# integritychain/fips204

Measured on AMD Instinct MI355X. Metric: ML-DSA-65 verifies/sec per GPU (batched); % HBM roofline, higher is better.
Workload: dtype int32; 1 GPU; ml_dsa_65 batch=65536 whole verify on FIPS 204 wire formats; batch_per_gpu=65536, parallelism=batch-split x1

## Files before the change

### fips204_amd/ml_dsa.py

```python
import ctypes as C

import numpy as np
import torch

from . import _keycheck_lib, _keys_lib, _lib, _mu_lib, _mus_lib, _ph_lib, _rec_lib, _seed_lib, _vfy_lib
from .hotpath import HotPath, N, _optr, _ptr, _stream

MODE_PURE, MODE_INTERNAL, MODE_PREHASH = 0, 1, 2

VFY_MIN_OPS = {44: 24576, 65: 16384, 87: 65536}

PH_SHA256, PH_SHA512, PH_SHAKE128 = "SHA256", "SHA512", "SHAKE128"
PH_SHA384, PH_SHA224, PH_SHA512_224, PH_SHA512_256 = "SHA384", "SHA224", "SHA512_224", "SHA512_256"
PH_SHA3_224, PH_SHA3_256, PH_SHA3_384, PH_SHA3_512, PH_SHAKE256 = "SHA3_224", "SHA3_256", "SHA3_384", "SHA3_512", "SHAKE256"
_PH_OID = bytes([0x06, 0x09, 0x60, 0x86, 0x48, 0x01, 0x65, 0x03, 0x04, 0x02])
_PH_TABLE = {
    PH_SHA256: (0x01, "sha256", None, _ph_lib.PH_SHA256),
    PH_SHA384: (0x02, "sha384", None, _ph_lib.PH_SHA384),
    PH_SHA512: (0x03, "sha512", None, _ph_lib.PH_SHA512),
    PH_SHA224: (0x04, "sha224", None, _ph_lib.PH_SHA224),
    PH_SHA512_224: (0x05, "sha512_224", None, _ph_lib.PH_SHA512_224),
    PH_SHA512_256: (0x06, "sha512_256", None, _ph_lib.PH_SHA512_256),
    PH_SHA3_224: (0x07, "sha3_224", None, _ph_lib.PH_SHA3_224),
    PH_SHA3_256: (0x08, "sha3_256", None, _ph_lib.PH_SHA3_256),
    PH_SHA3_384: (0x09, "sha3_384", None, _ph_lib.PH_SHA3_384),
    PH_SHA3_512: (0x0A, "sha3_512", None, _ph_lib.PH_SHA3_512),
    PH_SHAKE128: (0x0B, "shake_128", 32, _ph_lib.PH_SHAKE128),
    PH_SHAKE256: (0x0C, "shake_256", 64, _ph_lib.PH_SHAKE256),
}
_PH_ABI = {name: row[3] for name, row in _PH_TABLE.items()}
_PH_NAMES = "Ph: " + ", ".join(_PH_TABLE)


def _ph_code(ph):
    if ph not in _PH_ABI:
        raise ValueError(_PH_NAMES)
    return _PH_ABI[ph]


def _check_prehash(prehash):
    if prehash not in ("host", "device"):
        raise ValueError('prehash: "host" or "device"')
    return prehash == "device"


class OsRng:

    def fill_bytes(self, n):
        import os
        return os.urandom(n)


def hash_message(message, ph):
    import hashlib
    message = bytes(message)
    if not isinstance(ph, str) or ph not in _PH_TABLE:
        raise ValueError(_PH_NAMES)
    oid_last, name, xof_len, _ = _PH_TABLE[ph]
    h = hashlib.new(name, message)
    return _PH_OID + bytes([oid_last]) + (h.digest(xof_len) if xof_len else h.digest())


def external_mu(tr, message, ctx=b"", mode=MODE_PURE):
    import hashlib
    tr, message, ctx = bytes(tr), bytes(message), bytes(ctx)
    if len(tr) != 64:
        raise ValueError("tr: 64 bytes expected")
    if mode == MODE_INTERNAL:
        m_prime = message
    elif mode in (MODE_PURE, MODE_PREHASH):
        if len(ctx) > 255:
            raise ValueError("ctx too long (at most 255 bytes)")
        m_prime = bytes([1 if mode == MODE_PREHASH else 0, len(ctx)]) + ctx + message
    else:
        raise ValueError("mode: MODE_PURE, MODE_INTERNAL or MODE_PREHASH")
    return hashlib.shake_256(tr + m_prime).digest(64)


FORM_SEED, FORM_EXPANDED, FORM_BOTH = "seed", "expanded", "both"


def private_key_forms(seed=None, expanded=None):
    if seed is None and expanded is None:
        raise ValueError("a private key needs a seed, an expanded key or both")
    for name, key in (("seed", seed), ("expanded key", expanded)):
        if key is not None and not isinstance(key, (bytes, bytearray, memoryview)):
            raise TypeError(f"{name}: bytes, bytearray or memoryview expected, not {type(key).__name__}")
    if seed is not None and memoryview(seed).nbytes != _seed_lib.SEED_LEN:
        raise ValueError(f"seed: {_seed_lib.SEED_LEN} bytes expected")
    if expanded is not None and memoryview(expanded).nbytes == 0:
        raise ValueError("expanded key: empty")
    if expanded is None:
        return FORM_SEED, "expand_seeds"
    if seed is None:
        return FORM_EXPANDED, "sk_expand"
    return FORM_BOTH, "check_then_expand"


_SK_SHAPE = {44: (4, 4, 2), 65: (6, 5, 4), 87: (8, 7, 2)}


def private_key_faults(pset, sk_bytes):
    if pset not in _SK_SHAPE:
        raise ValueError(f"unknown parameter set {pset!r}")
    k, l, eta = _SK_SHAPE[pset]
    bits = 3 if eta == 2 else 4
    sk_len = 128 + 32 * bits * (l + k) + 416 * k
    if isinstance(sk_bytes, (bytes, bytearray, memoryview)):
        sk_bytes = [sk_bytes]
    if isinstance(sk_bytes, np.ndarray):
        a = np.ascontiguousarray(sk_bytes, dtype=np.uint8).reshape(-1)
    else:
        a = np.frombuffer(b"".join(bytes(b) for b in sk_bytes), dtype=np.uint8)
    if a.size % sk_len:
        raise ValueError(f"sk: {a.size} bytes are not a multiple of SK_LEN = {sk_len}")
    a = a.reshape(-1, sk_len)
    region = np.unpackbits(a[:, 128:128 + 32 * bits * (l + k)], axis=1, bitorder="little")
    fields = region.reshape(a.shape[0], (l + k) * 256, bits).astype(np.uint8) @ (1 << np.arange(bits)).astype(np.uint8)
    over = fields > 2 * eta
    return (over[:, :l * 256].any(axis=1) * _keycheck_lib.KEY_S1_RANGE + over[:, l * 256:].any(axis=1) * _keycheck_lib.KEY_S2_RANGE).astype(np.uint8)


def _np_ptr(a):
    return C.c_void_p(0) if a is None else C.c_void_p(a.ctypes.data)


def _cat(items):
    lens = np.fromiter((len(b) for b in items), dtype=np.uint64, count=len(items))
    off = np.zeros(len(items) + 1, dtype=np.uint64)
    np.cumsum(lens, out=off[1:])
    return b"".join(bytes(b) for b in items) or b"\0", off


def _cat_with_offsets(items, device):
    flat, off = _cat(items)
    buf = torch.frombuffer(bytearray(flat), dtype=torch.uint8).to(device)
    return buf, torch.from_numpy(off.view(np.int64)).to(device)


class PublicKeys:

    def __init__(self, pset, rho, tr, t1_d2_hat_mont):
        self.pset, self.rho, self.tr, self.t1_d2_hat_mont = pset, rho, tr, t1_d2_hat_mont

    def __len__(self):
        return self.rho.shape[0]


class PrivateKeys:

    def __init__(self, pset, rho, cap_k, tr, s_1_hat_mont, s_2_hat_mont, t_0_hat_mont):
        self.pset, self.rho, self.cap_k, self.tr = pset, rho, cap_k, tr
        self.s_1_hat_mont, self.s_2_hat_mont, self.t_0_hat_mont = s_1_hat_mont, s_2_hat_mont, t_0_hat_mont

    def __len__(self):
        return self.rho.shape[0]

    def zeroize(self):
        for t in (self.cap_k, self.s_1_hat_mont, self.s_2_hat_mont, self.t_0_hat_mont):
            if t is not None:
                t.zero_()

    def __del__(self):
# ... 1078 lines not shown
```

### fips204_amd/vfy/keccak180.h

```cpp
#pragma once
#include "../csrc/keccak.h"
#include "../csrc/sampler_dev.h"

namespace mldsa_vfy {

using mldsa::KeccakState;

#define VFY_RHOPI(DST, SRC, ROT)                                                                                                  \
    mldsa::rotl64<ROT>(mldsa::xor3(s.lo[SRC], clo[((SRC) + 4) % 5], rlo[((SRC) + 1) % 5]),                                        \
                       mldsa::xor3(s.hi[SRC], chi_[((SRC) + 4) % 5], rhi[((SRC) + 1) % 5]), blo[DST], bhi[DST])

__device__ __forceinline__ void keccak_round180(KeccakState& s, uint32_t rc_lo, uint32_t rc_hi) {
    uint32_t clo[5], chi_[5], rlo[5], rhi[5], blo[25], bhi[25];
#pragma unroll
    for (int x = 0; x < 5; x++) {
        clo[x] = mldsa::xor3(mldsa::xor3(s.lo[x], s.lo[x + 5], s.lo[x + 10]), s.lo[x + 15], s.lo[x + 20]);
        chi_[x] = mldsa::xor3(mldsa::xor3(s.hi[x], s.hi[x + 5], s.hi[x + 10]), s.hi[x + 15], s.hi[x + 20]);
    }
#pragma unroll
    for (int x = 0; x < 5; x++) mldsa::rotl64<1>(clo[x], chi_[x], rlo[x], rhi[x]);
    VFY_RHOPI(0, 0, 0);
    VFY_RHOPI(10, 1, 1);
    VFY_RHOPI(20, 2, 62);
    VFY_RHOPI(5, 3, 28);
    VFY_RHOPI(15, 4, 27);
    VFY_RHOPI(16, 5, 36);
    VFY_RHOPI(1, 6, 44);
    VFY_RHOPI(11, 7, 6);
    VFY_RHOPI(21, 8, 55);
    VFY_RHOPI(6, 9, 20);
    VFY_RHOPI(7, 10, 3);
    VFY_RHOPI(17, 11, 10);
    VFY_RHOPI(2, 12, 43);
    VFY_RHOPI(12, 13, 25);
    VFY_RHOPI(22, 14, 39);
    VFY_RHOPI(23, 15, 41);
    VFY_RHOPI(8, 16, 45);
    VFY_RHOPI(18, 17, 15);
    VFY_RHOPI(3, 18, 21);
    VFY_RHOPI(13, 19, 8);
    VFY_RHOPI(14, 20, 18);
    VFY_RHOPI(24, 21, 2);
    VFY_RHOPI(9, 22, 61);
    VFY_RHOPI(19, 23, 56);
    VFY_RHOPI(4, 24, 14);
#pragma unroll
    for (int y = 0; y < 25; y += 5) {
#pragma unroll
        for (int x = 0; x < 5; x++) {
            s.lo[y + x] = mldsa::chi(blo[y + x], blo[y + (x + 1) % 5], blo[y + (x + 2) % 5]);
            s.hi[y + x] = mldsa::chi(bhi[y + x], bhi[y + (x + 1) % 5], bhi[y + (x + 2) % 5]);
        }
    }
    s.lo[0] ^= rc_lo;
    s.hi[0] ^= rc_hi;
}
#undef VFY_RHOPI

__device__ __forceinline__ void keccak_f1600_180(KeccakState& s) {
#pragma unroll 1
    for (int r = 0; r < 24; r++) {
        const uint32_t rc_lo = mldsa::KECCAK_RC_LO[r];
        const uint32_t rc_hi = ((mldsa::KECCAK_RC_HI_BITS >> r) & 1u) << 31;
        keccak_round180(s, rc_lo, rc_hi);
    }
}

__device__ __forceinline__ void rej_ntt_poly_lane_direct180(KeccakState& st, int32_t* __restrict__ out, size_t wave_base, int lane, bool valid) {
    constexpr uint32_t ROW = mldsa::PACKED_POLY_DWORDS * 4;
    const size_t wb = ((size_t)(uint32_t)__builtin_amdgcn_readfirstlane((int)(wave_base >> 32)) << 32) |
                      (uint32_t)__builtin_amdgcn_readfirstlane((int)(uint32_t)wave_base);
    uint8_t* base = reinterpret_cast<uint8_t*>(out) + wb * ROW;
    const uint32_t end = (uint32_t)(lane + 1) * ROW;
    uint32_t off = valid ? (uint32_t)lane * ROW : end;
    while (__any(off < end)) {
        keccak_f1600_180(st);
        mldsa::static_for<0, 14>([&](auto gc) {
            constexpr int G = decltype(gc)::value;
            const uint32_t m0 = mldsa::state_word<3 * G>(st) & 0xFF7FFFFFu, m1 = mldsa::state_word<3 * G + 1>(st) & 0xFFFF7FFFu,
                           m2 = mldsa::state_word<3 * G + 2>(st) & 0x7FFFFF7Fu;
            const uint64_t lo = (((uint64_t)m1 << 32) | m0) + 0x1FFF001FFF001FFFull;
            const uint32_t hi = m2 + 0x001FFF00u + (uint32_t)(lo < 0x1FFF001FFF001FFFull ? 1u : 0u);
            const uint32_t over = ((uint32_t)lo & 0x00800000u) | ((uint32_t)(lo >> 32) & 0x00008000u) | (hi & 0x80000080u);
            if (over == 0u && off + 12u <= end) {
                *reinterpret_cast<mldsa::Packed3Unaligned*>(base + off) = mldsa::Packed3Unaligned{m0, m1, m2};
                off += 12u;
            } else if (off < end) {
                const uint32_t c[4] = {m0 & 0x7FFFFFu, __builtin_amdgcn_alignbit(m1, m0, 24) & 0x7FFFFFu,
                                       __builtin_amdgcn_alignbit(m2, m1, 16) & 0x7FFFFFu, m2 >> 8};
#pragma unroll
                for (int k = 0; k < 4; k++) {
                    if (c[k] < (uint32_t)mldsa::Q && off < end) {
                        uint8_t* dst = base + off;
                        dst[0] = (uint8_t)c[k];
                        dst[1] = (uint8_t)(c[k] >> 8);
                        dst[2] = (uint8_t)(c[k] >> 16);
                        off += 3u;
                    }
                }
            }
        });
    }
}

}
```

### fips204_amd/vfy/vfy.hip

```cpp
#include <hip/hip_runtime.h>
#include <stdint.h>
#include <string.h>

#include <mutex>
#include <string>
#include <vector>

#include "../../include/mldsa_vfy.h"
#include "../layer/layer_dev.h"
#include "../layer/layer_host.h"
#include "../csrc/challenge_dev.h"
#include "../csrc/ntt_wave.h"
#include "../csrc/sampler_dev.h"
#include "../csrc/tables.h"
#include "../csrc/verify_dev.h"
#include "keccak180.h"
#include "vfy_parts.h"

namespace mldsa_vfy {

using mldsa::FWD_TW;
using mldsa::INV_TW;
using mldsa::N;
using mldsa::SHAKE256_RATE;
// ... 404 lines not shown
        diff |= (st.lo[W] ^ load_le32(c0 + 8 * W)) | (st.hi[W] ^ load_le32(c0 + 8 * W + 4));
    });
    ok[op] = (uint8_t)(diff == 0 && znorm[op] < zbound && hvalid[op] && !ctx_bad[op]);
}

}

namespace {

using namespace mldsa_layer;
using namespace mldsa_vfy;

struct DevState {
    int dev = -1;
    int n_cu = 256;
    hipStream_t ea = nullptr, vm = nullptr;
    std::vector<hipEvent_t> ev;
    Twiddle *fwd = nullptr, *inv = nullptr;
    bool prof_on = false;
    std::vector<hipEvent_t> prof_ev;
    std::vector<const char*> prof_name;
    size_t prof_used = 0;
};

std::mutex g_mutex;
std::vector<DevState*> g_states;
size_t g_part_ops = 0;

size_t part_ops() { return g_part_ops ? g_part_ops : (size_t)MLDSA_VFY_PART_OPS; }

int dev_state(const char* fn, int dev, DevState** out) {
    for (DevState* d : g_states)
        if (d->dev == dev) {
            *out = d;
            return MLDSA_OK;
        }
    DevState* d = new DevState;
    d->dev = dev;
    int cu = 0;
    if (hipDeviceGetAttribute(&cu, hipDeviceAttributeMultiprocessorCount, dev) == hipSuccess && cu > 0) d->n_cu = cu;
    const std::vector<mldsa::HostTwiddle> f = mldsa::gen_fwd_lane_twiddles(), i = mldsa::gen_inv_lane_twiddles();
    hipError_t e = hipStreamCreateWithFlags(&d->ea, hipStreamNonBlocking);
    if (e == hipSuccess) e = hipStreamCreateWithFlags(&d->vm, hipStreamNonBlocking);
    if (e == hipSuccess) e = hipMalloc(&d->fwd, f.size() * sizeof(Twiddle));
    if (e == hipSuccess) e = hipMalloc(&d->inv, i.size() * sizeof(Twiddle));
    if (e == hipSuccess) e = hipMemcpy(d->fwd, f.data(), f.size() * sizeof(Twiddle), hipMemcpyHostToDevice);
    if (e == hipSuccess) e = hipMemcpy(d->inv, i.data(), i.size() * sizeof(Twiddle), hipMemcpyHostToDevice);
    if (e != hipSuccess || f.size() != (size_t)FWD_TW * 64 || i.size() != (size_t)INV_TW * 64) {
        if (d->ea) (void)hipStreamDestroy(d->ea);
        if (d->vm) (void)hipStreamDestroy(d->vm);
        if (d->fwd) (void)hipFree(d->fwd);
        if (d->inv) (void)hipFree(d->inv);
        delete d;
        (void)hipGetLastError();
        return e != hipSuccess ? hip_failed(fn, "creating the library's streams and tables", e)
                               : fail(MLDSA_ERR_DEVICE, std::string(fn) + ": the core's twiddle tables have another shape");
    }
    g_states.push_back(d);
    *out = d;
    return MLDSA_OK;
}

struct Events {
    DevState* d;
    size_t used = 0;
    hipError_t err = hipSuccess;
    explicit Events(DevState* d_) : d(d_) {}
    hipEvent_t next() {
        if (used == d->ev.size()) {
            hipEvent_t e = nullptr;
            const hipError_t rc = hipEventCreateWithFlags(&e, hipEventDisableTiming);
            if (rc != hipSuccess) {
                err = rc;
                return nullptr;
            }
            d->ev.push_back(e);
        }
        return d->ev[used++];
    }
};

constexpr size_t PROF_MAX_PAIRS = 4096;
struct ProfScope {
    DevState* d;
    hipStream_t s;
    long idx = -1;
    ProfScope(DevState* d_, hipStream_t s_, const char* name) : d(d_), s(s_) {
        if (!d->prof_on || d->prof_used >= PROF_MAX_PAIRS) return;
        if (d->prof_used * 2 + 2 > d->prof_ev.size()) {
            hipEvent_t a = nullptr, b = nullptr;
            if (hipEventCreate(&a) != hipSuccess) return;
            if (hipEventCreate(&b) != hipSuccess) {
                (void)hipEventDestroy(a);
                return;
            }
            d->prof_ev.push_back(a);
            d->prof_ev.push_back(b);
            d->prof_name.push_back(name);
        } else {
            d->prof_name[d->prof_used] = name;
        }
        idx = (long)d->prof_used++;
        (void)hipEventRecord(d->prof_ev[2 * idx], s);
    }
    ~ProfScope() {
        if (idx >= 0) (void)hipEventRecord(d->prof_ev[2 * idx + 1], s);
    }
};

#define VFY_HIP(call, what)                                     \
    do {                                                        \
        const hipError_t e_ = (call);                           \
        if (e_ != hipSuccess) return hip_failed(fn, what, e_);  \
    } while (0)

#define VFY_BY_SET(set, M)              \
    do {                                \
        if ((set) == MLDSA_44) M(4, 4, 17, false, 32, 5); \
        else if ((set) == MLDSA_65) M(6, 5, 19, true, 48, 4); \
        else M(8, 7, 19, true, 64, 4);  \
    } while (0)

unsigned stream_blocks(size_t n_streams) { return (unsigned)((n_streams + 64 * SWAVES - 1) / (64 * SWAVES)); }

void launch_expand_a(int set, const uint8_t* rho, const uint32_t* key_idx, int32_t* a_hat, size_t n, uint32_t n_keys, hipStream_t s) {
    mldsa_params p;
    (void)mldsa_get_params(set, &p);
    const dim3 grid(stream_blocks(n * (size_t)(p.k * p.l))), block(64 * SWAVES);
#define VFY_EA(KK, LL, GB, G2, CT, MW) hipLaunchKernelGGL((k_expand_a<KK, LL>), grid, block, 0, s, rho, (size_t)32, key_idx, a_hat, n, n_keys)
    VFY_BY_SET(set, VFY_EA);
#undef VFY_EA
}

struct Call {
    int set, mode;
    mldsa_params p;
    const uint8_t *rho, *tr;
    const int32_t* t1;
    size_t n_keys;
    const uint32_t* key_idx;
    const uint8_t* msgs;
    const uint64_t* msg_off;
    const uint8_t* ctxs;
    const uint64_t* ctx_off;
    const uint8_t* sigs;
    uint8_t* ok;
    size_t n_ops;
};

int enqueue(const char* fn, DevState* d, const Call& c, uint8_t* scratch, hipStream_t s) {
    const mldsa_params& p = c.p;
    const PartPlan plan(c.n_ops, part_ops());
    const Carve cv = carve(p.k, p.l, (size_t)p.w1_len, plan);
    const size_t mw = 64 + (size_t)p.w1_len, n_parts = plan.n_parts();
    uint32_t* c8 = reinterpret_cast<uint32_t*>(scratch + cv.c);
    int32_t* znorm = reinterpret_cast<int32_t*>(scratch + cv.znorm);
    int32_t* hvalid = reinterpret_cast<int32_t*>(scratch + cv.hvalid);
    int32_t* ctx_bad = reinterpret_cast<int32_t*>(scratch + cv.ctx_bad);
    int32_t* key_bad = reinterpret_cast<int32_t*>(scratch + cv.key_bad);
    uint32_t* kidx = reinterpret_cast<uint32_t*>(scratch + cv.kidx);
    uint8_t* mu_w1 = scratch + cv.mu_w1;
    const size_t sig_len = (size_t)p.sig_len;

    Events evs(d);
    hipEvent_t fork = evs.next(), join = evs.next();
    std::vector<hipEvent_t> ready(n_parts), used(n_parts), front(n_parts);
    for (size_t i = 0; i < n_parts; i++) {
        ready[i] = evs.next();
        used[i] = evs.next();
        front[i] = evs.next();
    }
    if (evs.err != hipSuccess) return hip_failed(fn, "creating an event", evs.err);

    VFY_HIP(hipEventRecord(fork, s), "recording the fork");
    VFY_HIP(hipStreamWaitEvent(d->ea, fork, 0), "ordering the ExpandA stream behind the caller's");
    VFY_HIP(hipStreamWaitEvent(d->vm, fork, 0), "ordering the arithmetic stream behind the caller's");
    for (size_t i = 0; i < n_parts; i++) {
        const Part part = plan.at(i);
        const size_t o = part.first, n = part.count;
        const size_t key_base = c.key_idx ? 0 : o;
        int32_t* a_hat = reinterpret_cast<int32_t*>(scratch + cv.ring[part.half]);
        const uint8_t* sg = c.sigs + o * sig_len;
        if (i >= 2) VFY_HIP(hipStreamWaitEvent(d->ea, used[i - 2], 0), "waiting for the ring half");
        {
            ProfScope ps(d, d->ea, "expand_a");
            launch_expand_a(c.set, c.rho + key_base * 32, c.key_idx ? c.key_idx + o : nullptr, a_hat, n, c.key_idx ? (uint32_t)c.n_keys : 0u, d->ea);
        }
        LAYER_LAUNCHED("k_expand_a launch");
        VFY_HIP(hipEventRecord(ready[i], d->ea), "recording ExpandA's end");
        const uint32_t* kp = nullptr;
        const int32_t* kb = nullptr;
        if (c.key_idx) {
            hipLaunchKernelGGL(k_sanitize_keys, dim3((unsigned)((n + 255) / 256)), dim3(256), 0, s, c.key_idx + o, (uint32_t)c.n_keys, n, kidx + o, key_bad + o);
            kp = kidx + o;
            kb = key_bad + o;
        }
        {
            ProfScope ps(d, s, "mu");
            hipLaunchKernelGGL(k_mu, dim3((unsigned)((n + 63) / 64)), dim3(64), 0, s, c.tr + key_base * 64, (size_t)64, kp, c.mode, c.msgs, c.msg_off, c.ctxs,
                               c.ctx_off, mu_w1 + o * mw, mw, ctx_bad + o, kb, n, o, c.n_ops);
        }
        {
            ProfScope ps(d, s, "sample_in_ball");
            const dim3 grid((unsigned)((n + 63) / 64)), block(64);
#define VFY_SIB(KK, LL, GB, G2, CT, MW) hipLaunchKernelGGL((k_sample_in_ball<CT>), grid, block, 0, s, sg, sig_len, p.tau, c8 + o * 64, n)
            VFY_BY_SET(c.set, VFY_SIB);
#undef VFY_SIB
        }
        LAYER_LAUNCHED("front launch");
        VFY_HIP(hipEventRecord(front[i], s), "recording the front's end");
        VFY_HIP(hipStreamWaitEvent(d->vm, ready[i], 0), "waiting for ExpandA");
        VFY_HIP(hipStreamWaitEvent(d->vm, front[i], 0), "waiting for the front");
        {
            ProfScope ps(d, d->vm, "verify_main");
            const size_t need = (n + VW - 1) / VW, cap = (size_t)d->n_cu * 16;
            const dim3 grid((unsigned)(need < cap ? need : cap)), block(64 * VW);
#define VFY_VM(KK, LL, GB, G2, CT, MW)                                                                                                         \
    hipLaunchKernelGGL((k_verify_main<KK, LL, GB, G2, MW>), grid, block, 0, d->vm, reinterpret_cast<const uint32_t*>(a_hat), sg, sig_len,      \
                       p.ctilde_len, c8 + o * 64, c.t1, kp, key_base, hvalid + o, p.omega, mu_w1 + o * mw + 64, mw, znorm + o, p.gamma1 - p.beta, n, \
                       d->fwd, d->inv)
            VFY_BY_SET(c.set, VFY_VM);
#undef VFY_VM
        }
        LAYER_LAUNCHED("k_verify_main launch");
        VFY_HIP(hipEventRecord(used[i], d->vm), "recording the end of the ring half's use");
        {
            ProfScope ps(d, d->vm, "ctilde_hash");
            const dim3 grid((unsigned)((n + CBLOCK - 1) / CBLOCK)), block(CBLOCK);
#define VFY_CT(KK, LL, GB, G2, CT, MW)                                                                                                    \
    hipLaunchKernelGGL((k_ctilde_verdict<CT>), grid, block, 0, d->vm, mu_w1 + o * mw, mw, sg, sig_len, znorm + o, p.gamma1 - p.beta, hvalid + o, \
                       ctx_bad + o, c.ok + o, n)
            VFY_BY_SET(c.set, VFY_CT);
#undef VFY_CT
        }
        LAYER_LAUNCHED("k_ctilde_verdict launch");
    }
    VFY_HIP(hipEventRecord(join, d->vm), "recording the join");
    VFY_HIP(hipStreamWaitEvent(s, join, 0), "joining the caller's stream");
    return MLDSA_OK;
}

void drain(DevState* d) {
    (void)hipStreamSynchronize(d->ea);
    (void)hipStreamSynchronize(d->vm);
    (void)hipGetLastError();
}

size_t scratch_bytes_of(int set, size_t n_ops) {
    mldsa_params p;
    if (mldsa_get_params(set, &p) != MLDSA_OK || n_ops > MLDSA_VFY_MAX_OPS) return 0;
    return carve(p.k, p.l, (size_t)p.w1_len, PartPlan(n_ops, part_ops())).bytes;
}

}

extern "C" {

int mldsa_vfy_abi_version(void) { return MLDSA_VFY_ABI_VERSION; }

const char* mldsa_vfy_last_error(void) { return g_err.c_str(); }

size_t mldsa_vfy_scratch_bytes(int set, size_t n_ops) {
    std::lock_guard<std::mutex> lk(g_mutex);
    return scratch_bytes_of(set, n_ops);
}

size_t mldsa_vfy_set_part_ops(size_t part) {
    std::lock_guard<std::mutex> lk(g_mutex);
    const size_t before = part_ops();
    g_part_ops = part;
    return before;
}

int mldsa_vfy_verify(mldsa_ctx* ctx, int set, int mode, const uint8_t* rho, const uint8_t* tr, const int32_t* t1_d2_hat_mont, size_t n_keys,
                     const uint32_t* key_idx, const uint8_t* msgs, const uint64_t* msg_off, const uint8_t* ctxs, const uint64_t* ctx_off,
                     const uint8_t* sigs, uint8_t* ok, size_t n_ops, void* scratch, size_t scratch_bytes, void* stream) {
    const char* fn = "mldsa_vfy_verify";
    Call c;
    const int rc = check_common(fn, ctx, set, n_ops, MLDSA_VFY_MAX_OPS, "MLDSA_VFY_MAX_OPS ops", &c.p);
    if (rc != MLDSA_OK) return rc;
    if (mode != MLDSA_MODE_PURE && mode != MLDSA_MODE_INTERNAL && mode != MLDSA_MODE_PREHASH)
        return fail(MLDSA_ERR_PARAM, std::string(fn) + ": bad mode");
    if (n_ops == 0) return MLDSA_OK;
    if (!rho || !tr || !t1_d2_hat_mont || !msg_off || !sigs || !ok) return fail(MLDSA_ERR_PARAM, std::string(fn) + ": NULL pointer");
    if (key_idx ? n_keys == 0 : n_keys < n_ops) return fail(MLDSA_ERR_PARAM, std::string(fn) + ": n_keys does not cover the batch");
    if (n_keys > 0xFFFFFFFFu) n_keys = 0xFFFFFFFFu;
    if (!aligned(t1_d2_hat_mont, 16)) return fail(MLDSA_ERR_PARAM, std::string(fn) + ": t1_d2_hat_mont must be 16-byte aligned");
    if (!scratch || !aligned(scratch, 256)) return fail(MLDSA_ERR_PARAM, std::string(fn) + ": scratch is NULL or not 256-byte aligned");
    LAYER_ON_DEVICE(ctx);
    std::lock_guard<std::mutex> lk(g_mutex);
    if (scratch_bytes < scratch_bytes_of(set, n_ops))
        return fail(MLDSA_ERR_NOMEM, std::string(fn) + ": scratch is below mldsa_vfy_scratch_bytes(set, n_ops)");
    DevState* d = nullptr;
    const int src = dev_state(fn, dev_, &d);
    if (src != MLDSA_OK) return src;
    c.set = set; c.mode = mode; c.rho = rho; c.tr = tr; c.t1 = t1_d2_hat_mont; c.n_keys = n_keys; c.key_idx = key_idx; c.msgs = msgs;
    c.msg_off = msg_off; c.ctxs = ctxs; c.ctx_off = ctx_off; c.sigs = sigs; c.ok = ok; c.n_ops = n_ops;
    const int erc = enqueue(fn, d, c, static_cast<uint8_t*>(scratch), (hipStream_t)stream);
    if (erc != MLDSA_OK) drain(d);
    return erc;
}

int mldsa_vfy_expand_a(mldsa_ctx* ctx, int set, const uint8_t* rho, int32_t* a_hat, size_t n_ops, void* stream) {
    const char* fn = "mldsa_vfy_expand_a";
    mldsa_params p;
    const int rc = check_common(fn, ctx, set, n_ops, MLDSA_VFY_MAX_OPS, "MLDSA_VFY_MAX_OPS ops", &p);
    if (rc != MLDSA_OK) return rc;
    if (n_ops == 0) return MLDSA_OK;
    if (!rho || !a_hat) return fail(MLDSA_ERR_PARAM, std::string(fn) + ": NULL pointer");
    if (!aligned(a_hat, 16)) return fail(MLDSA_ERR_PARAM, std::string(fn) + ": a_hat must be 16-byte aligned");
    LAYER_ON_DEVICE(ctx);
    hipStream_t s = (hipStream_t)stream;
    const size_t n_polys = n_ops * (size_t)(p.k * p.l);
    void* packed = nullptr;
    VFY_HIP(hipMalloc(&packed, n_polys * PACKED_POLY_BYTES), "allocating the packed rows");
    launch_expand_a(set, rho, nullptr, static_cast<int32_t*>(packed), n_ops, 0u, s);
    hipLaunchKernelGGL(k_unpack_a, dim3((unsigned)((n_polys + 3) / 4)), dim3(256), 0, s, static_cast<const uint32_t*>(packed), a_hat, n_polys);
    hipError_t e = hipGetLastError();
    const hipError_t se = hipStreamSynchronize(s);
    if (e == hipSuccess) e = se;
    (void)hipFree(packed);
    return e == hipSuccess ? MLDSA_OK : hip_failed(fn, "ExpandA and unpack", e);
}

int mldsa_vfy_profile_enable(mldsa_ctx* ctx, int on) {
    const char* fn = "mldsa_vfy_profile_enable";
    if (!ctx) return fail(MLDSA_ERR_PARAM, std::string(fn) + ": NULL context");
    LAYER_ON_DEVICE(ctx);
    std::lock_guard<std::mutex> lk(g_mutex);
    DevState* d = nullptr;
    const int rc = dev_state(fn, dev_, &d);
    if (rc != MLDSA_OK) return rc;
    d->prof_on = on != 0;
    if (!d->prof_on) d->prof_used = 0;
    return MLDSA_OK;
}

int mldsa_vfy_profile_report(mldsa_ctx* ctx, char* buf, size_t buf_len) {
    const char* fn = "mldsa_vfy_profile_report";
    if (!ctx) return fail(MLDSA_ERR_PARAM, std::string(fn) + ": NULL context");
    if (!buf || buf_len <= 2) return fail(MLDSA_ERR_PARAM, std::string(fn) + ": bad argument");
    LAYER_ON_DEVICE(ctx);
    std::lock_guard<std::mutex> lk(g_mutex);
    DevState* d = nullptr;
    const int rc = dev_state(fn, dev_, &d);
    if (rc != MLDSA_OK) return rc;
    VFY_HIP(hipDeviceSynchronize(), "waiting for the device");
    struct Acc { const char* name; double ms; size_t calls; };
    std::vector<Acc> acc;
    for (size_t i = 0; i < d->prof_used; i++) {
        float ms = 0.f;
        if (hipEventElapsedTime(&ms, d->prof_ev[2 * i], d->prof_ev[2 * i + 1]) != hipSuccess) {
            (void)hipGetLastError();
            continue;
        }
        bool found = false;
        for (auto& a : acc)
            if (strcmp(a.name, d->prof_name[i]) == 0) {
                a.ms += ms;
                a.calls++;
                found = true;
                break;
            }
        if (!found) acc.push_back({d->prof_name[i], ms, 1});
    }
    std::string out = "{";
    for (size_t i = 0; i < acc.size(); i++)
        out += std::string(i ? ", " : "") + "\"" + acc[i].name + "\": {\"ms\": " + std::to_string(acc[i].ms) + ", \"calls\": " + std::to_string(acc[i].calls) + "}";
    out += "}";
    if (out.size() + 1 > buf_len) return fail(MLDSA_ERR_PARAM, std::string(fn) + ": buffer too small");
    memcpy(buf, out.c_str(), out.size() + 1);
    d->prof_used = 0;
    return MLDSA_OK;
}

}
```

### fips204_amd/vfy/vfy_parts.h

```cpp
#pragma once
#include <stddef.h>
#include <stdint.h>

namespace mldsa_vfy {

constexpr size_t PACKED_POLY_BYTES = 768;
constexpr size_t CARVE_ALIGN = 256;

struct Part {
    size_t first = 0, count = 0;
    int half = 0;
};

struct PartPlan {
    size_t n_ops, part;
    PartPlan(size_t n_ops_, size_t part_) : n_ops(n_ops_), part(part_ ? part_ : 1) {}
    size_t n_parts() const { return n_ops / part + (n_ops % part ? 1 : 0); }
    size_t halves() const { return n_parts() > 1 ? 2 : n_parts(); }
    size_t half_ops() const { return n_ops < part ? n_ops : part; }
    Part at(size_t i) const {
        Part p;
        p.first = i * part;
        p.count = n_ops - p.first < part ? n_ops - p.first : part;
        p.half = (int)(i & 1);
        return p;
    }
};

struct Carve {
    size_t ring[2];
    size_t ring_bytes;
    size_t c;
    size_t znorm, hvalid, ctx_bad, key_bad, kidx;
    size_t mu_w1;
    size_t bytes;
};

inline size_t carve_up(size_t x) { return (x + CARVE_ALIGN - 1) / CARVE_ALIGN * CARVE_ALIGN; }

inline Carve carve(int k, int l, size_t w1_len, const PartPlan& plan) {
    Carve c;
    size_t at = 0;
    auto take = [&at](size_t bytes) {
        const size_t here = at;
        at += carve_up(bytes);
        return here;
    };
    c.ring_bytes = plan.half_ops() * (size_t)(k * l) * PACKED_POLY_BYTES;
    c.ring[0] = take(c.ring_bytes);
    c.ring[1] = plan.halves() > 1 ? take(c.ring_bytes) : c.ring[0];
    c.c = take(plan.n_ops * 256);
    c.znorm = take(plan.n_ops * 4);
    c.hvalid = take(plan.n_ops * 4);
    c.ctx_bad = take(plan.n_ops * 4);
    c.key_bad = take(plan.n_ops * 4);
    c.kidx = take(plan.n_ops * 4);
    c.mu_w1 = take(plan.n_ops * (64 + w1_len));
    c.bytes = at + CARVE_ALIGN;
    return c;
}

}
```

Measured before the change: 40.24 million verifies/s.

## Restructure rejection sampler with unconditional head blocks and shifted-compare acceptance test

Splits the per-lane rejection sampler for the NTT-domain matrix into a fixed head of four Keccak blocks and a tail loop. The head needs no end-of-row bounds checks or wave-wide __any votes, because four blocks can never fill a row, and it uses constant-offset stores with a bias. The acceptance test becomes a max over left-shifted 23-bit candidates compared against Q<<8, replacing the 64-bit carry trick, and byte stores become a 16-bit plus an 8-bit store. It also lowers the ML-DSA-87 minimum batch threshold for the verify path, which does not affect the ML-DSA-65 workload.

```diff
diff --git a/fips204_amd/ml_dsa.py b/fips204_amd/ml_dsa.py
--- a/fips204_amd/ml_dsa.py
+++ b/fips204_amd/ml_dsa.py
@@ -8,7 +8,7 @@
 
 MODE_PURE, MODE_INTERNAL, MODE_PREHASH = 0, 1, 2
 
-VFY_MIN_OPS = {44: 24576, 65: 16384, 87: 65536}
+VFY_MIN_OPS = {44: 24576, 65: 16384, 87: 49152}
 
 PH_SHA256, PH_SHA512, PH_SHAKE128 = "SHA256", "SHA512", "SHAKE128"
 PH_SHA384, PH_SHA224, PH_SHA512_224, PH_SHA512_256 = "SHA384", "SHA224", "SHA512_224", "SHA512_256"
diff --git a/fips204_amd/vfy/keccak180.h b/fips204_amd/vfy/keccak180.h
--- a/fips204_amd/vfy/keccak180.h
+++ b/fips204_amd/vfy/keccak180.h
@@ -66,35 +66,62 @@
     }
 }
 
+struct __attribute__((packed, aligned(1))) Packed2Unaligned { uint16_t v; };
+
+__device__ __forceinline__ void store_coeff3(uint8_t* dst, uint32_t t) {
+    const uint32_t c = t >> 8;
+    *reinterpret_cast<Packed2Unaligned*>(dst) = Packed2Unaligned{(uint16_t)c};
+    dst[2] = (uint8_t)(c >> 16);
+}
+
 __device__ __forceinline__ void rej_ntt_poly_lane_direct180(KeccakState& st, int32_t* __restrict__ out, size_t wave_base, int lane, bool valid) {
     constexpr uint32_t ROW = mldsa::PACKED_POLY_DWORDS * 4;
+    constexpr uint32_t HEAD_BIAS = 256;
+    constexpr int HEAD_BLOCKS = 4;
+    constexpr uint32_t QT = (uint32_t)mldsa::Q << 8;
     const size_t wb = ((size_t)(uint32_t)__builtin_amdgcn_readfirstlane((int)(wave_base >> 32)) << 32) |
                       (uint32_t)__builtin_amdgcn_readfirstlane((int)(uint32_t)wave_base);
     uint8_t* base = reinterpret_cast<uint8_t*>(out) + wb * ROW;
+    const uint32_t thr = valid ? QT : 0u;
+    uint32_t off = (uint32_t)lane * ROW + HEAD_BIAS;
+#pragma unroll 1
+    for (int b = 0; b < HEAD_BLOCKS; b++) {
+        keccak_f1600_180(st);
+        mldsa::static_for<0, 14>([&](auto gc) {
+            constexpr int G = decltype(gc)::value;
+            constexpr ptrdiff_t AT = 12 * G - (ptrdiff_t)HEAD_BIAS;
+            const uint32_t m0 = mldsa::state_word<3 * G>(st) & 0xFF7FFFFFu, m1 = mldsa::state_word<3 * G + 1>(st) & 0xFFFF7FFFu,
+                           m2 = mldsa::state_word<3 * G + 2>(st) & 0x7FFFFF7Fu;
+            const uint32_t t[4] = {m0 << 8, __builtin_amdgcn_alignbit(m1, m0, 16), __builtin_amdgcn_alignbit(m2, m1, 8), m2};
+            if (max(max(t[0], t[1]), max(t[2], t[3])) < thr) {
+                *reinterpret_cast<mldsa::Packed3Unaligned*>(base + (size_t)off + AT) = mldsa::Packed3Unaligned{m0, m1, m2};
+            } else {
+#pragma unroll
+                for (int k = 0; k < 4; k++) {
+                    if (t[k] < thr) store_coeff3(base + (size_t)off + (AT + 3 * k), t[k]);
+                    else off -= 3u;
+                }
+            }
+        });
+        off += 168u;
+    }
     const uint32_t end = (uint32_t)(lane + 1) * ROW;
-    uint32_t off = valid ? (uint32_t)lane * ROW : end;
+    off = valid ? off - HEAD_BIAS : end;
     while (__any(off < end)) {
         keccak_f1600_180(st);
         mldsa::static_for<0, 14>([&](auto gc) {
             constexpr int G = decltype(gc)::value;
             const uint32_t m0 = mldsa::state_word<3 * G>(st) & 0xFF7FFFFFu, m1 = mldsa::state_word<3 * G + 1>(st) & 0xFFFF7FFFu,
                            m2 = mldsa::state_word<3 * G + 2>(st) & 0x7FFFFF7Fu;
-            const uint64_t lo = (((uint64_t)m1 << 32) | m0) + 0x1FFF001FFF001FFFull;
-            const uint32_t hi = m2 + 0x001FFF00u + (uint32_t)(lo < 0x1FFF001FFF001FFFull ? 1u : 0u);
-            const uint32_t over = ((uint32_t)lo & 0x00800000u) | ((uint32_t)(lo >> 32) & 0x00008000u) | (hi & 0x80000080u);
-            if (over == 0u && off + 12u <= end) {
+            const uint32_t t[4] = {m0 << 8, __builtin_amdgcn_alignbit(m1, m0, 16), __builtin_amdgcn_alignbit(m2, m1, 8), m2};
+            if (max(max(t[0], t[1]), max(t[2], t[3])) < QT && off + 12u <= end) {
                 *reinterpret_cast<mldsa::Packed3Unaligned*>(base + off) = mldsa::Packed3Unaligned{m0, m1, m2};
                 off += 12u;
             } else if (off < end) {
-                const uint32_t c[4] = {m0 & 0x7FFFFFu, __builtin_amdgcn_alignbit(m1, m0, 24) & 0x7FFFFFu,
-                                       __builtin_amdgcn_alignbit(m2, m1, 16) & 0x7FFFFFu, m2 >> 8};
 #pragma unroll
                 for (int k = 0; k < 4; k++) {
-                    if (c[k] < (uint32_t)mldsa::Q && off < end) {
-                        uint8_t* dst = base + off;
-                        dst[0] = (uint8_t)c[k];
-                        dst[1] = (uint8_t)(c[k] >> 8);
-                        dst[2] = (uint8_t)(c[k] >> 16);
+                    if (t[k] < QT && off < end) {
+                        store_coeff3(base + off, t[k]);
                         off += 3u;
                     }
                 }
```

Measured after the change: 40.41 million verifies/s (median of 6 runs). About the same (+0.4%).

## Drive stage launches from a computed stream/event order plan, collapsing lanes for single-part calls

Applied to the files above, without the earlier changes.

Replaces the hard-coded per-part fork/ready/front/used/join event scheme with a generated step plan that records and waits on events only when producer and consumer sit on different streams. When the call has only one part, ExpandA and the arithmetic stages run on the caller's stream and only the front runs on a side stream, which removes most cross-stream event records and waits. Multi-part calls keep the same three-lane overlap. The aim is to cut event and stream-wait overhead, at the cost of less concurrency between ExpandA and verify in the single-part case.

```diff
diff --git a/fips204_amd/vfy/vfy.hip b/fips204_amd/vfy/vfy.hip
--- a/fips204_amd/vfy/vfy.hip
+++ b/fips204_amd/vfy/vfy.hip
@@ -580,7 +580,7 @@
     const mldsa_params& p = c.p;
     const PartPlan plan(c.n_ops, part_ops());
     const Carve cv = carve(p.k, p.l, (size_t)p.w1_len, plan);
-    const size_t mw = 64 + (size_t)p.w1_len, n_parts = plan.n_parts();
+    const size_t mw = 64 + (size_t)p.w1_len;
     uint32_t* c8 = reinterpret_cast<uint32_t*>(scratch + cv.c);
     int32_t* znorm = reinterpret_cast<int32_t*>(scratch + cv.znorm);
     int32_t* hvalid = reinterpret_cast<int32_t*>(scratch + cv.hvalid);
@@ -590,81 +590,78 @@
     uint8_t* mu_w1 = scratch + cv.mu_w1;
     const size_t sig_len = (size_t)p.sig_len;
 
+    const OrderPlan order = order_plan(plan.n_parts());
+    const hipStream_t lanes[N_LANES] = {s, d->ea, d->vm};
     Events evs(d);
-    hipEvent_t fork = evs.next(), join = evs.next();
-    std::vector<hipEvent_t> ready(n_parts), used(n_parts), front(n_parts);
-    for (size_t i = 0; i < n_parts; i++) {
-        ready[i] = evs.next();
-        used[i] = evs.next();
-        front[i] = evs.next();
-    }
+    std::vector<hipEvent_t> ev(order.n_events);
+    for (hipEvent_t& e : ev) e = evs.next();
     if (evs.err != hipSuccess) return hip_failed(fn, "creating an event", evs.err);
 
-    VFY_HIP(hipEventRecord(fork, s), "recording the fork");
-    VFY_HIP(hipStreamWaitEvent(d->ea, fork, 0), "ordering the ExpandA stream behind the caller's");
-    VFY_HIP(hipStreamWaitEvent(d->vm, fork, 0), "ordering the arithmetic stream behind the caller's");
-    for (size_t i = 0; i < n_parts; i++) {
-        const Part part = plan.at(i);
+    for (const Step& st : order.steps) {
+        const hipStream_t q = lanes[st.lane];
+        if (st.act == ACT_RECORD) {
+            VFY_HIP(hipEventRecord(ev[st.n], q), (std::string("recording ") + st.what).c_str());
+            continue;
+        }
+        if (st.act == ACT_WAIT) {
+            VFY_HIP(hipStreamWaitEvent(q, ev[st.n], 0), (std::string("waiting for ") + st.what).c_str());
+            continue;
+        }
+        const Part part = plan.at(st.n);
         const size_t o = part.first, n = part.count;
         const size_t key_base = c.key_idx ? 0 : o;
         int32_t* a_hat = reinterpret_cast<int32_t*>(scratch + cv.ring[part.half]);
         const uint8_t* sg = c.sigs + o * sig_len;
-        if (i >= 2) VFY_HIP(hipStreamWaitEvent(d->ea, used[i - 2], 0), "waiting for the ring half");
-        {
-            ProfScope ps(d, d->ea, "expand_a");
-            launch_expand_a(c.set, c.rho + key_base * 32, c.key_idx ? c.key_idx + o : nullptr, a_hat, n, c.key_idx ? (uint32_t)c.n_keys : 0u, d->ea);
-        }
-        LAYER_LAUNCHED("k_expand_a launch");
-        VFY_HIP(hipEventRecord(ready[i], d->ea), "recording ExpandA's end");
-        const uint32_t* kp = nullptr;
-        const int32_t* kb = nullptr;
-        if (c.key_idx) {
-            hipLaunchKernelGGL(k_sanitize_keys, dim3((unsigned)((n + 255) / 256)), dim3(256), 0, s, c.key_idx + o, (uint32_t)c.n_keys, n, kidx + o, key_bad + o);
-            kp = kidx + o;
-            kb = key_bad + o;
-        }
-        {
-            ProfScope ps(d, s, "mu");
-            hipLaunchKernelGGL(k_mu, dim3((unsigned)((n + 63) / 64)), dim3(64), 0, s, c.tr + key_base * 64, (size_t)64, kp, c.mode, c.msgs, c.msg_off, c.ctxs,
-                               c.ctx_off, mu_w1 + o * mw, mw, ctx_bad + o, kb, n, o, c.n_ops);
-        }
-        {
-            ProfScope ps(d, s, "sample_in_ball");
-            const dim3 grid((unsigned)((n + 63) / 64)), block(64);
-#define VFY_SIB(KK, LL, GB, G2, CT, MW) hipLaunchKernelGGL((k_sample_in_ball<CT>), grid, block, 0, s, sg, sig_len, p.tau, c8 + o * 64, n)
-            VFY_BY_SET(c.set, VFY_SIB);
+        const uint32_t* kp = c.key_idx ? kidx + o : nullptr;
+        const int32_t* kb = c.key_idx ? key_bad + o : nullptr;
+        switch (st.stage) {
+        case STAGE_EXPAND_A: {
+            ProfScope ps(d, q, "expand_a");
+            launch_expand_a(c.set, c.rho + key_base * 32, c.key_idx ? c.key_idx + o : nullptr, a_hat, n, c.key_idx ? (uint32_t)c.n_keys : 0u, q);
+            break;
+        }
+        case STAGE_FRONT: {
+            if (c.key_idx)
+                hipLaunchKernelGGL(k_sanitize_keys, dim3((unsigned)((n + 255) / 256)), dim3(256), 0, q, c.key_idx + o, (uint32_t)c.n_keys, n, kidx + o, key_bad + o);
+            {
+                ProfScope ps(d, q, "mu");
+                hipLaunchKernelGGL(k_mu, dim3((unsigned)((n + 63) / 64)), dim3(64), 0, q, c.tr + key_base * 64, (size_t)64, kp, c.mode, c.msgs, c.msg_off, c.ctxs,
+                                   c.ctx_off, mu_w1 + o * mw, mw, ctx_bad + o, kb, n, o, c.n_ops);
+            }
+            {
+                ProfScope ps(d, q, "sample_in_ball");
+                const dim3 grid((unsigned)((n + 63) / 64)), block(64);
+#define VFY_SIB(KK, LL, GB, G2, CT, MW) hipLaunchKernelGGL((k_sample_in_ball<CT>), grid, block, 0, q, sg, sig_len, p.tau, c8 + o * 64, n)
+                VFY_BY_SET(c.set, VFY_SIB);
 #undef VFY_SIB
-        }
-        LAYER_LAUNCHED("front launch");
-        VFY_HIP(hipEventRecord(front[i], s), "recording the front's end");
-        VFY_HIP(hipStreamWaitEvent(d->vm, ready[i], 0), "waiting for ExpandA");
-        VFY_HIP(hipStreamWaitEvent(d->vm, front[i], 0), "waiting for the front");
-        {
-            ProfScope ps(d, d->vm, "verify_main");
+            }
+            break;
+        }
+        case STAGE_VERIFY_MAIN: {
+            ProfScope ps(d, q, "verify_main");
             const size_t need = (n + VW - 1) / VW, cap = (size_t)d->n_cu * 16;
             const dim3 grid((unsigned)(need < cap ? need : cap)), block(64 * VW);
 #define VFY_VM(KK, LL, GB, G2, CT, MW)                                                                                                         \
-    hipLaunchKernelGGL((k_verify_main<KK, LL, GB, G2, MW>), grid, block, 0, d->vm, reinterpret_cast<const uint32_t*>(a_hat), sg, sig_len,      \
+    hipLaunchKernelGGL((k_verify_main<KK, LL, GB, G2, MW>), grid, block, 0, q, reinterpret_cast<const uint32_t*>(a_hat), sg, sig_len,          \
                        p.ctilde_len, c8 + o * 64, c.t1, kp, key_base, hvalid + o, p.omega, mu_w1 + o * mw + 64, mw, znorm + o, p.gamma1 - p.beta, n, \
                        d->fwd, d->inv)
             VFY_BY_SET(c.set, VFY_VM);
 #undef VFY_VM
-        }
-        LAYER_LAUNCHED("k_verify_main launch");
-        VFY_HIP(hipEventRecord(used[i], d->vm), "recording the end of the ring half's use");
-        {
-            ProfScope ps(d, d->vm, "ctilde_hash");
+            break;
+        }
+        default: {
+            ProfScope ps(d, q, "ctilde_hash");
             const dim3 grid((unsigned)((n + CBLOCK - 1) / CBLOCK)), block(CBLOCK);
 #define VFY_CT(KK, LL, GB, G2, CT, MW)                                                                                                    \
-    hipLaunchKernelGGL((k_ctilde_verdict<CT>), grid, block, 0, d->vm, mu_w1 + o * mw, mw, sg, sig_len, znorm + o, p.gamma1 - p.beta, hvalid + o, \
+    hipLaunchKernelGGL((k_ctilde_verdict<CT>), grid, block, 0, q, mu_w1 + o * mw, mw, sg, sig_len, znorm + o, p.gamma1 - p.beta, hvalid + o, \
                        ctx_bad + o, c.ok + o, n)
             VFY_BY_SET(c.set, VFY_CT);
 #undef VFY_CT
-        }
-        LAYER_LAUNCHED("k_ctilde_verdict launch");
-    }
-    VFY_HIP(hipEventRecord(join, d->vm), "recording the join");
-    VFY_HIP(hipStreamWaitEvent(s, join, 0), "joining the caller's stream");
+            break;
+        }
+        }
+        LAYER_LAUNCHED(st.what);
+    }
     return MLDSA_OK;
 }
 
diff --git a/fips204_amd/vfy/vfy_parts.h b/fips204_amd/vfy/vfy_parts.h
--- a/fips204_amd/vfy/vfy_parts.h
+++ b/fips204_amd/vfy/vfy_parts.h
@@ -1,6 +1,8 @@
 #pragma once
 #include <stddef.h>
 #include <stdint.h>
+
+#include <vector>
 
 namespace mldsa_vfy {
 
@@ -60,4 +62,72 @@
     return c;
 }
 
+enum Lane { LANE_CALLER = 0, LANE_EA = 1, LANE_VM = 2, N_LANES = 3 };
+enum Action { ACT_RECORD, ACT_WAIT, ACT_LAUNCH };
+enum Stage { STAGE_EXPAND_A = 0, STAGE_FRONT = 1, STAGE_VERIFY_MAIN = 2, STAGE_CTILDE = 3, N_STAGES = 4 };
+
+struct Step {
+    Lane lane;
+    Action act;
+    Stage stage;
+    size_t n;
+    const char* what;
+};
+
+struct OrderPlan {
+    std::vector<Step> steps;
+    size_t n_events = 0;
+};
+
+struct StageLanes {
+    Lane expand_a, arith, front;
+};
+inline StageLanes lanes_of_call(size_t n_parts) {
+    return n_parts == 1 ? StageLanes{LANE_CALLER, LANE_CALLER, LANE_VM} : StageLanes{LANE_EA, LANE_VM, LANE_CALLER};
 }
+
+inline OrderPlan order_plan(size_t n_parts, const StageLanes& on) {
+    OrderPlan o;
+    if (n_parts == 0) return o;
+    const size_t none = (size_t)-1;
+    auto put = [&o](Lane lane, Action act, Stage stage, size_t n, const char* what) { o.steps.push_back(Step{lane, act, stage, n, what}); };
+    const size_t fork = o.n_events++;
+    bool forked[N_LANES] = {true, false, false};
+    auto reach = [&](Lane lane, Stage stage) {
+        if (!forked[lane]) put(lane, ACT_WAIT, stage, fork, "the fork");
+        forked[lane] = true;
+    };
+    auto record = [&](Lane from, Lane to, Stage stage, const char* what) {
+        if (from == to) return none;
+        put(from, ACT_RECORD, stage, o.n_events, what);
+        return o.n_events++;
+    };
+    auto wait = [&](Lane to, size_t event, Stage stage, const char* what) {
+        if (event == none) return;
+        put(to, ACT_WAIT, stage, event, what);
+        forked[to] = true;
+    };
+    put(LANE_CALLER, ACT_RECORD, STAGE_EXPAND_A, fork, "the fork");
+    std::vector<size_t> used(n_parts, none);
+    for (size_t p = 0; p < n_parts; p++) {
+        if (p >= 2) wait(on.expand_a, used[p - 2], STAGE_EXPAND_A, "the ring half");
+        reach(on.expand_a, STAGE_EXPAND_A);
+        put(on.expand_a, ACT_LAUNCH, STAGE_EXPAND_A, p, "k_expand_a launch");
+        const size_t ready = record(on.expand_a, on.arith, STAGE_EXPAND_A, "ExpandA's end");
+        reach(on.front, STAGE_FRONT);
+        put(on.front, ACT_LAUNCH, STAGE_FRONT, p, "front launch");
+        const size_t front = record(on.front, on.arith, STAGE_FRONT, "the front's end");
+        wait(on.arith, ready, STAGE_EXPAND_A, "ExpandA");
+        wait(on.arith, front, STAGE_FRONT, "the front");
+        reach(on.arith, STAGE_VERIFY_MAIN);
+        put(on.arith, ACT_LAUNCH, STAGE_VERIFY_MAIN, p, "k_verify_main launch");
+        if (p + 2 < n_parts) used[p] = record(on.arith, on.expand_a, STAGE_VERIFY_MAIN, "the end of the ring half's use");
+        put(on.arith, ACT_LAUNCH, STAGE_CTILDE, p, "k_ctilde_verdict launch");
+    }
+    wait(LANE_CALLER, record(on.arith, LANE_CALLER, STAGE_CTILDE, "the join"), STAGE_CTILDE, "the join");
+    return o;
+}
+
+inline OrderPlan order_plan(size_t n_parts) { return order_plan(n_parts, lanes_of_call(n_parts)); }
+
+}
```

New measurement: 40.47 million verifies/s before, 41.00 million verifies/s after, median of 6. +1.3%, better.
